# quokka-astro/quokka

Measured on AMD Instinct MI355X. Metric: Mcell-updates/s on 3D Sedov unigrid, higher is better.
Workload: dtype f64; 1 GPU; 3D Sedov blast 256x256x256 unigrid (tests/blast_unigrid_256.in scaled to 256^3 cells per GPU), 128^3 boxes, PPM+HLLC RK2, gamma=1.4, CFL 0.3, reflecting octant; cells_per_gpu=16777216, boxes_per_gpu=8, parallelism=box-decomposition x1, rk2_mode=carry, fofc_stages=0, retries=0, x_sweep_in_y_march=True

## Files before the change

include/quokka_amd.h:

```cpp
#ifndef QUOKKA_AMD_H_
#define QUOKKA_AMD_H_

#include <stdint.h>

#ifdef __cplusplus
extern "C" {
#endif

typedef struct qk_ctx qk_ctx;
typedef struct qk_level qk_level;
typedef void *qk_stream;

typedef enum qk_status {
	QK_OK = 0,
	QK_ERR_INVALID = -1,
	QK_ERR_HIP = -2,
	QK_ERR_UNSUPPORTED = -3,
	QK_ERR_STATE = -4
} qk_status;

typedef struct qk_array4 {
	double *p;
	int64_t jstride, kstride, nstride;
	int begin[3];
// ... 202 lines not shown
int qk_ghost_plan_destroy(qk_ghost_plan *plan);
int qk_ghost_plan_num_peers(qk_ghost_plan *plan);
int qk_ghost_plan_peer(qk_ghost_plan *plan, int k, int *rank, int64_t *send_count, int64_t *recv_count);
int qk_ghost_plan_num_items(qk_ghost_plan *plan, int kind, int k);
int qk_ghost_plan_item(qk_ghost_plan *plan, int kind, int k, int idx, int *dst_box, int *src_box, int lo[3], int hi[3], int shift[3], int64_t *offset);
int qk_FillBoundary_local(qk_ghost_plan *plan, qk_stream s, qk_array4 *state);
int qk_FillBoundary_local_int(qk_ghost_plan *plan, qk_stream s, qk_iarray4 *state);
int qk_FillBoundary_pack(qk_ghost_plan *plan, qk_stream s, int k, const qk_array4 *state, double *sendbuf);
int qk_FillBoundary_unpack(qk_ghost_plan *plan, qk_stream s, int k, qk_array4 *state, const double *recvbuf);
int qk_FillBoundary_pack_int(qk_ghost_plan *plan, qk_stream s, int k, const qk_iarray4 *state, int *sendbuf);
int qk_FillBoundary_unpack_int(qk_ghost_plan *plan, qk_stream s, int k, qk_iarray4 *state, const int *recvbuf);
int qk_SumBoundary_local(qk_ghost_plan *plan, qk_stream s, qk_array4 *state);
int qk_SumBoundary_pack(qk_ghost_plan *plan, qk_stream s, int k, const qk_array4 *state, double *buf);
int qk_SumBoundary_unpack(qk_ghost_plan *plan, qk_stream s, int k, qk_array4 *state, const double *buf);
int qk_FillPhysicalBoundary(qk_ghost_plan *plan, qk_stream s, qk_array4 *state, const qk_bcrec *bcs, const qk_dirichlet_face *dirichlet);
int qk_ghost_plan_set_components(qk_ghost_plan *plan, int scomp, int ncomp);
#define QK_BOXES_ALL 0
#define QK_BOXES_LOCAL_ONLY 1
#define QK_BOXES_REMOTE_DEPENDENT 2
int qk_ghost_plan_box_is_remote(qk_ghost_plan *plan, int local_box);
int qk_ghost_plan_set_box_remote(qk_ghost_plan *plan, int local_box, int flag);
int qk_FillPhysicalBoundary_subset(qk_ghost_plan *plan, qk_stream s, qk_array4 *state, const qk_bcrec *bcs, const qk_dirichlet_face *dirichlet,
				   int which);

typedef struct qk_carray4 {
	char *p;
	int64_t jstride, kstride, nstride;
	int begin[3];
	int end[3];
	int ncomp;
} qk_carray4;
enum { QK_TAG_CLEAR = 0, QK_TAG_BUF = 1, QK_TAG_SET = 2 };
#define QK_TAGFIELD_PRESSURE (-1)
int qk_tag_relative_gradient(qk_level *lev, qk_stream s, const qk_hydro_traits *t, const qk_array4 *state, qk_carray4 *tags, int field,
			     double eta_threshold, double q_min, int min_inclusive);
int qk_tag_centered_gradient(qk_level *lev, qk_stream s, const qk_array4 *state, qk_carray4 *tags, int comp, int dir, double dx, double eta_threshold,
			     double q_min, int min_inclusive);
int qk_PreInterpState(qk_level *lev, qk_stream s, qk_array4 *mf);
int qk_PostInterpState(qk_level *lev, qk_stream s, qk_array4 *mf);
typedef struct qk_avgdown_plan qk_avgdown_plan;
int qk_avgdown_plan_create(qk_level *crse, qk_level *fine, const int ratio[3], qk_avgdown_plan **plan);
int qk_avgdown_plan_destroy(qk_avgdown_plan *plan);
int qk_avgdown_plan_num_items(qk_avgdown_plan *plan);
int qk_average_down(qk_avgdown_plan *plan, qk_stream s, const qk_array4 *fine, qk_array4 *crse, int scomp, int ncomp);

typedef struct qk_interp_plan qk_interp_plan;
// ... 82 lines not shown
```

quokka_amd/capi.py:

```python
from __future__ import annotations

import ctypes as C
import os

_HERE = os.path.dirname(os.path.abspath(__file__))
LIB_PATH = os.environ.get("QK_LIB_PATH", os.path.join(_HERE, "lib", "libquokka_amd.so"))

QK_OK, QK_ERR_INVALID, QK_ERR_HIP, QK_ERR_UNSUPPORTED, QK_ERR_STATE = 0, -1, -2, -3, -4
ERR_UNSUPPORTED = QK_ERR_UNSUPPORTED
HOOK_COMPILED = 100
DIR_X1, DIR_X2, DIR_X3 = 0, 1, 2
ARITH_DIVBY_RECIPOF, ARITH_DIVN, ARITH_RECIPEXACT, ARITH_SQRTN = 0, 1, 2, 3
RIEMANN_HLLC, RIEMANN_LLF, RIEMANN_HLLD = 0, 1, 2
LIMITER_MINMOD, LIMITER_MC = 0, 1
BC_REFLECT_ODD, BC_INT_DIR, BC_REFLECT_EVEN, BC_FOEXTRAP, BC_EXT_DIR = -1, 0, 1, 2, 3

K_B = 1.380649e-16
M_U = 1.6605390666e-24


class Array4(C.Structure):
    _fields_ = [("p", C.c_void_p), ("jstride", C.c_int64), ("kstride", C.c_int64), ("nstride", C.c_int64),
                ("begin", C.c_int * 3), ("end", C.c_int * 3), ("ncomp", C.c_int)]

# ... 46 lines not shown
        for g in range(ng + 1):
            self.rad_boundaries[g] = float(boundaries[g])
            self.mg_kappa_exponent[g] = float(kappa_exponent[g])
            self.mg_kappa_lower[g] = float(kappa_lower[g])
        self.mg_kappa_rho_exponent, self.mg_kappa_T_ref, self.mg_kappa_T_exponent = float(rho_exponent), float(T_ref), float(T_exponent)
        return self


class CloudyTables(C.Structure):
    _fields_ = [("log_nH", C.c_void_p), ("log_Tgas", C.c_void_p), ("cooling", C.c_void_p), ("heating", C.c_void_p), ("mean_mol_weight", C.c_void_p),
                ("n_nH", C.c_int), ("n_Tgas", C.c_int), ("T_min", C.c_double), ("T_max", C.c_double), ("mmw_min", C.c_double), ("mmw_max", C.c_double)]


class StageArgs(C.Structure):
    _fields_ = [("U_in", C.c_void_p), ("U_old", C.c_void_p), ("U_out", C.c_void_p),
                ("halfFlux", C.c_void_p * 3), ("halfVel", C.c_void_p * 3),
                ("redoFlag", C.c_void_p), ("d_redo_count", C.c_void_p), ("d_error_flag", C.c_void_p), ("d_max_signal", C.c_void_p),
                ("scratch", C.c_void_p), ("scratch_bytes", C.c_int64),
                ("dx", C.c_double * 3), ("dt", C.c_double), ("stage", C.c_int), ("reconstruction_order", C.c_int),
                ("densityFloor", C.c_double), ("tempFloor", C.c_double), ("use_dual_energy", C.c_int), ("K_visc", C.c_double),
                ("store_flux_rk2", C.c_int), ("fluxRk2", C.c_void_p * 3), ("rk2_carry_rhs", C.c_int), ("rhs1", C.c_void_p), ("flux_mask", C.c_void_p), ("fofc_pass", C.c_int),
                ("prim_out", C.c_int), ("prim_in", C.c_int),
                ("store_vel_rk2", C.c_int), ("velRk2", C.c_void_p * 3)]


def traits(gamma=1.4, reconstruct_eint=True, ndim=3, mean_molecular_weight=M_U, boltzmann_constant=K_B,
           cs_isothermal=float("nan"), nscalars=0, nmscalars=0, eos_temperature_model=0, eos_alpha=0.0) -> HydroTraits:
    return HydroTraits(gamma, cs_isothermal, mean_molecular_weight, boltzmann_constant, int(reconstruct_eint), nscalars, nmscalars, ndim,
                       int(eos_temperature_model), float(eos_alpha))


class QkError(RuntimeError):
    pass


_lib = None


def lib() -> C.CDLL:
    global _lib
    if _lib is not None:
        return _lib
    if not os.path.exists(LIB_PATH):
        raise QkError(f"{LIB_PATH} is missing: run `python -c 'import __graft_entry__ as g; g.build()'` "
                      "(hipcc --offload-arch=gfx950). The hot path has no CPU fallback.")
    L = C.CDLL(LIB_PATH)
# ... 33 lines not shown
    L.qk_hydro_EnforceLimits.argtypes = [vp, vp, T, cd, cd, vp]
    L.qk_hydro_SyncDualEnergy.argtypes = [vp, vp, T, vp, vp]
    L.qk_hydro_ComputeMaxSignalSpeed.argtypes = [vp, vp, T, vp, vp]
    L.qk_hydro_maxSignalSpeedLocal.argtypes = [vp, vp, T, ci, vp, vp]
    L.qk_replaceFluxes.argtypes = [vp, vp, ci, vp, vp, vp, ci]
    L.qk_Saxpy.argtypes = [vp, vp, ci, vp, cd, vp, ci]
    R = P(RadTraits)
    L.qk_rad_ConservedToPrimitive.argtypes = [vp, vp, R, vp, vp, ci]
    L.qk_rad_ComputeFluxes.argtypes = [vp, vp, R, ci, vp, vp, vp, vp, vp]
    L.qk_rad_computeRadiationFluxes.argtypes = [vp, vp, R, ci, ci, vp, P(vp), P(vp)]
    L.qk_rad_ComputeWavespeedCorrection.argtypes = [vp, vp, R, T, ci, vp, P(cd), P(vp)]
    L.qk_rad_PredictStep.argtypes = [vp, vp, R, ci, vp, vp, P(vp), cd, P(cd)]
    L.qk_rad_AddFluxesRK2.argtypes = [vp, vp, R, ci, vp, vp, vp, P(vp), P(vp), cd, P(cd)]
    L.qk_hydro_FixupState.argtypes = [vp, vp, T, cd, cd, ci, vp, vp, vp]
    L.qk_rad_stage_fused.argtypes = [vp, vp, R, ci, ci, vp, vp, vp, vp, P(vp), cd, P(cd), P(vp)]
    L.qk_rad_AddSourceTermsSingleGroup.argtypes = [vp, vp, R, T, vp, vp, cd, ci, vp, vp]
    L.qk_rad_AddSourceTermsSingleGroupMirror.argtypes = [vp, vp, R, T, vp, vp, cd, ci, vp, vp, vp]
    L.qk_rad_AddSourceTermsMultiGroup.argtypes = [vp, vp, R, T, vp, vp, cd, ci, vp, vp]
    L.qk_rad_mg_planck_fractions.argtypes = [vp, R, cd, ci, P(cd), P(cd), P(cd)]
    if hasattr(L, "qk_hydro_stage_fused"):
        L.qk_hydro_stage_scratch_bytes.argtypes = [vp, T]
        L.qk_hydro_stage_scratch_bytes.restype = C.c_int64
        L.qk_hydro_stage_fused.argtypes = [vp, vp, T, P(StageArgs)]
    if hasattr(L, "qk_ghost_plan_create"):
        L.qk_ghost_plan_create.argtypes = [vp, P(vp), P(Geometry), ci, ci, ci, P(Box), P(ci), ci]
        L.qk_ghost_plan_destroy.argtypes = [vp]
        L.qk_ghost_plan_num_peers.argtypes = [vp]
        L.qk_ghost_plan_peer.argtypes = [vp, ci, P(ci), P(C.c_int64), P(C.c_int64)]
        L.qk_ghost_plan_num_items.argtypes = [vp, ci, ci]
        L.qk_ghost_plan_item.argtypes = [vp, ci, ci, ci, P(ci), P(ci), ci * 3, ci * 3, ci * 3, P(C.c_int64)]
        L.qk_FillBoundary_local.argtypes = [vp, vp, vp]
        L.qk_FillBoundary_local_int.argtypes = [vp, vp, vp]
        L.qk_FillBoundary_pack.argtypes = [vp, vp, ci, vp, vp]
        L.qk_FillBoundary_unpack.argtypes = [vp, vp, ci, vp, vp]
        L.qk_SumBoundary_local.argtypes = [vp, vp, vp]
        L.qk_SumBoundary_pack.argtypes = [vp, vp, ci, vp, vp]
        L.qk_SumBoundary_unpack.argtypes = [vp, vp, ci, vp, vp]
        L.qk_FillBoundary_pack_int.argtypes = [vp, vp, ci, vp, vp]
        L.qk_FillBoundary_unpack_int.argtypes = [vp, vp, ci, vp, vp]
        L.qk_FillPhysicalBoundary.argtypes = [vp, vp, vp, P(BCRec), P(DirichletFace)]
        L.qk_FillPhysicalBoundary_subset.argtypes = [vp, vp, vp, P(BCRec), P(DirichletFace), C.c_int]
        L.qk_ghost_plan_set_components.argtypes = [vp, C.c_int, C.c_int]
        L.qk_ghost_plan_box_is_remote.argtypes = [vp, C.c_int]
        L.qk_ghost_plan_set_box_remote.argtypes = [vp, C.c_int, C.c_int]
    if hasattr(L, "qk_tag_relative_gradient"):
        L.qk_tag_relative_gradient.argtypes = [vp, vp, T, vp, vp, ci, C.c_double, C.c_double, ci]
# ... 26 lines not shown
        L.qk_PreInterpState.argtypes = [vp, vp, vp]
        L.qk_PostInterpState.argtypes = [vp, vp, vp]
        L.qk_fluxreg_create_crse_part.argtypes = [vp, vp, P(Geometry), ci * 3, ci, P(vp)]
        L.qk_pcopy_plan_create.argtypes = [vp, P(Geometry), ci, P(Box), P(ci), ci, ci, ci, P(Box), P(ci), ci, vp, ci, ci, P(vp)]
        L.qk_pcopy_plan_destroy.argtypes = [vp]
        L.qk_pcopy_plan_num_peers.argtypes = [vp]
        L.qk_pcopy_plan_peer.argtypes = [vp, ci, P(ci), P(C.c_int64), P(C.c_int64)]
        L.qk_pcopy_plan_num_items.argtypes = [vp, ci, ci]
        L.qk_pcopy_plan_item.argtypes = [vp, ci, ci, ci, P(ci), P(ci), ci * 3, ci * 3, ci * 3, P(C.c_int64)]
        L.qk_ParallelCopy_local.argtypes = [vp, vp, vp, vp, ci, ci, ci]
        L.qk_ParallelCopy_pack.argtypes = [vp, vp, ci, vp, ci, vp]
        L.qk_ParallelCopy_unpack.argtypes = [vp, vp, ci, vp, ci, vp, ci]
    L.qk_tracer_plan_create.argtypes = [vp, P(vp), P(Geometry), cd * 3, cd * 3, cd * 3]
    L.qk_tracer_plan_destroy.argtypes = [vp]
    L.qk_tracer_plan_lattice.argtypes = [vp, ci * 3, P(C.c_int64)]
    L.qk_tracer_InitOnePerCell.argtypes = [vp, vp, cd * 3, vp * 3, vp * 3, vp, vp, C.c_int64, ci]
    L.qk_tracer_AdvectWithUmac.argtypes = [vp, vp, vp * 3, cd, C.c_int64, vp * 3, vp * 3]
    L.qk_tracer_Redistribute.argtypes = [vp, vp, C.c_int64, vp * 3, vp]
    _lib = L
    return L


BOXES_ALL, BOXES_LOCAL_ONLY, BOXES_REMOTE_DEPENDENT = 0, 1, 2
TAG_CLEAR, TAG_BUF, TAG_SET = 0, 1, 2
TAGFIELD_PRESSURE = -1

DECLARED_SYMBOLS = [
    "qk_ctx_create", "qk_ctx_destroy", "qk_last_error", "qk_version", "qk_level_create", "qk_level_destroy",
    "qk_upload_array4_table", "qk_upload_iarray4_table", "qk_clear_bytes", "qk_profile_enable", "qk_profile_only", "qk_profile_reset", "qk_profile_num_kernels", "qk_profile_get",
    "qk_ReconstructStatesConstant", "qk_ReconstructStatesPLM", "qk_ReconstructStatesPPM",
    "qk_hydro_ConservedToPrimitive", "qk_hydro_ComputeFlatteningCoefficients", "qk_hydro_FlattenShocks",
    "qk_hydro_ComputeFluxes", "qk_hydro_ComputeRhsFromFluxes", "qk_hydro_AddInternalEnergyPdV", "qk_hydro_PredictStep",
    "qk_hydro_EnforceLimits", "qk_hydro_SyncDualEnergy", "qk_hydro_ComputeMaxSignalSpeed", "qk_hydro_maxSignalSpeedLocal",
    "qk_replaceFluxes", "qk_Saxpy", "qk_hydro_FixupState", "qk_hydro_stage_scratch_bytes", "qk_hydro_stage_fused",
    "qk_rad_ConservedToPrimitive", "qk_rad_ComputeWavespeedCorrection", "qk_rad_ComputeFluxes", "qk_rad_computeRadiationFluxes", "qk_rad_PredictStep", "qk_rad_AddFluxesRK2", "qk_rad_stage_fused",
    "qk_rad_AddSourceTermsSingleGroup", "qk_rad_AddSourceTermsSingleGroupMirror", "qk_rad_AddSourceTermsMultiGroup", "qk_rad_mg_planck_fractions",
    "qk_ghost_plan_create", "qk_ghost_plan_destroy", "qk_ghost_plan_num_peers", "qk_ghost_plan_peer", "qk_ghost_plan_num_items", "qk_ghost_plan_item",
    "qk_FillBoundary_local", "qk_FillBoundary_local_int", "qk_FillBoundary_pack", "qk_FillBoundary_unpack", "qk_FillBoundary_pack_int", "qk_FillBoundary_unpack_int", "qk_SumBoundary_local", "qk_SumBoundary_pack", "qk_SumBoundary_unpack", "qk_FillPhysicalBoundary",
    "qk_FillPhysicalBoundary_subset", "qk_ghost_plan_set_components", "qk_ghost_plan_box_is_remote", "qk_ghost_plan_set_box_remote",
    "qk_tag_relative_gradient", "qk_tag_centered_gradient", "qk_avgdown_plan_create", "qk_avgdown_plan_destroy", "qk_avgdown_plan_num_items", "qk_average_down", "qk_PreInterpState", "qk_PostInterpState",
    "qk_interp_plan_create", "qk_interp_plan_destroy", "qk_interp_plan_num_items", "qk_interp_plan_item", "qk_InterpFromCoarse",
    "qk_fluxreg_create", "qk_fluxreg_destroy", "qk_fluxreg_num_items", "qk_fluxreg_item", "qk_fluxreg_reset", "qk_fluxreg_save", "qk_fluxreg_restore", "qk_fluxreg_CrseAdd", "qk_fluxreg_FineAdd",
    "qk_fluxreg_Reflux", "qk_fluxreg_set_state_component", "qk_amr_tile_flags", "qk_amr_tile_flags_periodic", "qk_amr_cluster_tiles", "qk_amr_cluster_berger_rigoutsos", "qk_copy_box",
    "qk_cloudy_tables_read", "qk_cloudy_tables_free", "qk_cooling_tabulated", "qk_cooling_evaluate", "qk_arith_evaluate",
    "qk_fluxreg_create_crse_part", "qk_pcopy_plan_create", "qk_pcopy_plan_destroy", "qk_pcopy_plan_num_peers", "qk_pcopy_plan_peer", "qk_pcopy_plan_num_items",
    "qk_pcopy_plan_item", "qk_ParallelCopy_local", "qk_ParallelCopy_pack", "qk_ParallelCopy_unpack",
    "qk_tracer_plan_create", "qk_tracer_plan_destroy", "qk_tracer_plan_lattice", "qk_tracer_InitOnePerCell", "qk_tracer_AdvectWithUmac", "qk_tracer_Redistribute",
]


def check(ctx, rc: int, what: str = "") -> None:
    if rc != QK_OK:
        msg = lib().qk_last_error(ctx).decode() if ctx else ""
        raise QkError(f"{what} failed with status {rc}: {msg}")
```

quokka_amd/csrc/qk_boundary.hip:

```cpp
#include <algorithm>
#include <cstdlib>
#include <array>
#include <map>
#include <cstring>
#include <vector>

#include "qk_device.hpp"
#include "qk_internal.hpp"

using namespace qk;

namespace
{

struct CopyItem {
	int dst_box;
	int src_box;
	int lo[3], hi[3];
	int shift[3];
	int64_t offset;
};

struct PeerPlan {
	int rank = -1;
// ... 9 lines not shown
}

}

struct qk_ghost_plan {
	qk_level *lev = nullptr;
	qk_geometry geom{};
	int nghost = 0, ncomp = 0;
	std::vector<CopyItem> local;
	CopyItem *d_local = nullptr;
	int max_local_cells = 0;
	std::vector<PeerPlan> peers;
	std::vector<CopyItem> shells;
	CopyItem *d_shells = nullptr;
	int max_shell_cells = 0;
	int n_shells_indep = 0;
	std::vector<char> box_remote;
	int active_scomp = 0, active_ncomp = -1;
	void *d_physbc = nullptr;
	std::vector<unsigned char> h_physbc;
	qk_bcrec *d_bcs = nullptr;
	int d_bcs_n = 0;
	qk_dirichlet_face *d_dir = nullptr;
};

namespace
{

void partitionShells(qk_ghost_plan *P)
{
	auto indep = [&](CopyItem const &it) { return P->box_remote[it.dst_box] == 0; };
	std::stable_partition(P->shells.begin(), P->shells.end(), indep);
	P->n_shells_indep = static_cast<int>(std::count_if(P->shells.begin(), P->shells.end(), indep));
}

enum CopyMode { MODE_LOCAL = 0, MODE_PACK = 1, MODE_UNPACK = 2, MODE_SUM_LOCAL = 3, MODE_SUM_PACK = 4, MODE_SUM_UNPACK = 5 };

template <int MODE, typename T = double, typename D = qk_array4>
__global__ void __launch_bounds__(256) k_copy(const CopyItem *items, const D *state_t, T *buf, int ncomp, int scomp = 0)
{
	const CopyItem it = items[blockIdx.y];
	const unsigned n0 = static_cast<unsigned>(it.hi[0] - it.lo[0] + 1), n1 = static_cast<unsigned>(it.hi[1] - it.lo[1] + 1),
		       n2 = static_cast<unsigned>(it.hi[2] - it.lo[2] + 1);
	const unsigned n01 = n0 * n1;
	const unsigned ncell = n01 * n2;
	const unsigned total = ncell * static_cast<unsigned>(ncomp);
// ... 129 lines not shown
			for (int d = 0; d < 3; ++d) {
				if (side[d] == 0) {
					continue;
				}
				const int type = (side[d] < 0) ? bc.lo[d] : bc.hi[d];
				const int edge = (side[d] < 0) ? geom.domain.lo[d] : geom.domain.hi[d];
				if (type == QK_BC_FOEXTRAP) {
					src[d] = edge;
					any = true;
				} else if (type == QK_BC_REFLECT_EVEN || type == QK_BC_REFLECT_ODD) {
					src[d] = (side[d] < 0) ? (2 * edge - idx[d] - 1) : (2 * edge - idx[d] + 1);
					neg = neg != (type == QK_BC_REFLECT_ODD);
					any = true;
				}
			}
			if (any) {
				const double v = A(src[0], src[1], src[2], n);
				A(idx[0], idx[1], idx[2], n) = neg ? -v : v;
			}
		}
	}
}

auto uploadItems(qk_ctx *ctx, std::vector<CopyItem> const &v, CopyItem **d) -> int
{
	*d = nullptr;
	if (v.empty() || ctx->device < 0) {
		return QK_OK;
	}
	QK_HIP_CHECK(ctx, hipMalloc(reinterpret_cast<void **>(d), sizeof(CopyItem) * v.size()));
	QK_HIP_CHECK(ctx, hipMemcpy(*d, v.data(), sizeof(CopyItem) * v.size(), hipMemcpyHostToDevice));
	return QK_OK;
}

inline auto gridFor(int64_t cells, int nitems) -> dim3
{
	const int64_t gx = std::max<int64_t>(1, std::min<int64_t>((cells + 255) / 256, 256));
	return dim3(static_cast<unsigned>(gx), static_cast<unsigned>(nitems), 1);
}
constexpr int MAX_ITEMS_PER_LAUNCH = 65535;

template <class Launch> void forItemChunks(int count, Launch &&launch)
{
	for (int a = 0; a < count; a += MAX_ITEMS_PER_LAUNCH) {
		launch(a, std::min(count - a, MAX_ITEMS_PER_LAUNCH));
	}
// ... 177 lines not shown
	}
	if (rc != QK_OK) {
		qk_ghost_plan_destroy(P);
		return rc;
	}
	*plan_out = P;
	return QK_OK;
}

int qk_ghost_plan_destroy(qk_ghost_plan *plan)
{
	if (plan == nullptr) {
		return QK_ERR_INVALID;
	}
	(void)hipFree(plan->d_local);
	(void)hipFree(plan->d_shells);
	for (auto &p : plan->peers) {
		(void)hipFree(p.d_send);
		(void)hipFree(p.d_recv);
	}
	(void)hipFree(plan->d_bcs);
	(void)hipFree(plan->d_dir);
	(void)hipFree(plan->d_physbc);
	delete plan;
	return QK_OK;
}

int qk_ghost_plan_num_peers(qk_ghost_plan *plan) { return plan == nullptr ? QK_ERR_INVALID : static_cast<int>(plan->peers.size()); }

int qk_ghost_plan_peer(qk_ghost_plan *plan, int k, int *rank, int64_t *send_count, int64_t *recv_count)
{
	if (plan == nullptr) {
		return QK_ERR_INVALID;
	}
	QK_REQUIRE(plan->lev->ctx, k >= 0 && k < static_cast<int>(plan->peers.size()) && rank && send_count && recv_count, "qk_ghost_plan_peer: bad index");
	*rank = plan->peers[k].rank;
	*send_count = plan->peers[k].send_count;
	*recv_count = plan->peers[k].recv_count;
	return QK_OK;
}

static auto planItems(qk_ghost_plan *plan, int kind, int k) -> std::vector<CopyItem> const *
{
	if (kind == 0) {
		return &plan->local;
	}
// ... 204 lines not shown
	QK_HIP_CHECK(ctx, hipGetLastError());
	return QK_OK;
}

int qk_ghost_plan_box_is_remote(qk_ghost_plan *plan, int local_box)
{
	if (plan == nullptr || local_box < 0 || local_box >= plan->lev->nboxes) {
		return QK_ERR_INVALID;
	}
	return plan->box_remote[local_box];
}

int qk_ghost_plan_set_box_remote(qk_ghost_plan *plan, int local_box, int flag)
{
	if (plan == nullptr || local_box < 0 || local_box >= plan->lev->nboxes) {
		return QK_ERR_INVALID;
	}
	qk_ctx *ctx = plan->lev->ctx;
	plan->box_remote[local_box] = (flag != 0) ? 1 : 0;
	partitionShells(plan);
	if (plan->d_shells != nullptr && !plan->shells.empty()) {
		QK_HIP_CHECK(ctx, hipMemcpy(plan->d_shells, plan->shells.data(), sizeof(CopyItem) * plan->shells.size(), hipMemcpyHostToDevice));
	}
	return QK_OK;
}

int qk_FillPhysicalBoundary(qk_ghost_plan *plan, qk_stream s, qk_array4 *state_t, const qk_bcrec *bcs, const qk_dirichlet_face *dirichlet)
{
	return qk_FillPhysicalBoundary_subset(plan, s, state_t, bcs, dirichlet, QK_BOXES_ALL);
}

int qk_ghost_plan_set_components(qk_ghost_plan *plan, int scomp, int ncomp)
{
	if (plan == nullptr) {
		return QK_ERR_INVALID;
	}
	QK_REQUIRE(plan->lev->ctx, ncomp < 0 || (scomp >= 0 && ncomp >= 1 && scomp + ncomp <= plan->ncomp), "ghost_plan_set_components: bad range");
	plan->active_scomp = (ncomp < 0) ? 0 : scomp;
	plan->active_ncomp = ncomp;
	return QK_OK;
}

int qk_FillPhysicalBoundary_subset(qk_ghost_plan *plan, qk_stream s, qk_array4 *state_t, const qk_bcrec *bcs, const qk_dirichlet_face *dirichlet,
				   int which)
{
	if (plan == nullptr) {
// ... 64 lines not shown
```

quokka_amd/simulation.py:

```python
from __future__ import annotations

import ctypes as C
import math
import os
from dataclasses import dataclass
from typing import Callable, List, Optional, Sequence, Tuple

import numpy as np
import torch

from . import capi
from .hydro_system import HydroSystem, HyperbolicSystem, Saxpy, replaceFluxes
from .multifab import Context, Level, MultiFab

NGHOST_CC = 4


def chop_domain(n_cell: Sequence[int], max_grid_size: Sequence[int]) -> List[Tuple[List[int], List[int]]]:
    nb = [(n_cell[d] + max_grid_size[d] - 1) // max_grid_size[d] for d in range(3)]
    boxes = []
    for kb in range(nb[2]):
        for jb in range(nb[1]):
            for ib in range(nb[0]):
                lo, hi = [], []
# ... 98 lines not shown
        self.peers = []
        for k in range(L.qk_ghost_plan_num_peers(h)):
            r, ns, nr = C.c_int(), C.c_int64(), C.c_int64()
            ctx.check(L.qk_ghost_plan_peer(h, k, C.byref(r), C.byref(ns), C.byref(nr)), "qk_ghost_plan_peer")
            self.peers.append((k, r.value, torch.empty(ns.value, dtype=dtype, device=ctx.device), torch.empty(nr.value, dtype=dtype, device=ctx.device)))

    def fill(self, state: MultiFab, between=None, before_physbc=None):
        ctx = self.lev.ctx
        L = ctx.L
        s = ctx.stream()
        def pack(k, sbuf):
            ctx.check(L.qk_FillBoundary_pack(self.h, s, k, state.ptr, C.c_void_p(sbuf.data_ptr())), "FillBoundary_pack")

        def local():
            ctx.check(L.qk_FillBoundary_local(self.h, s, state.ptr), "FillBoundary_local")

        def unpack(k, rbuf):
            ctx.check(L.qk_FillBoundary_unpack(self.h, s, k, state.ptr, C.c_void_p(rbuf.data_ptr())), "FillBoundary_unpack")

        def physbc(which):
            ctx.check(L.qk_FillPhysicalBoundary_subset(self.h, s, state.ptr, self.bcs, self.dirichlet, which), "FillPhysicalBoundary")

        self.fill_with(pack, local, unpack, physbc, between, before_physbc)

    def fill_with(self, pack, local, unpack, physbc, between=None, before_physbc=None):
        pending = None
        if self.peers:
            from . import comm
            for k, r, sbuf, rbuf in self.peers:
                pack(k, sbuf)
            pending = comm.exchange([(r, sbuf, rbuf) for k, r, sbuf, rbuf in self.peers])
        local()
        bc = not self.geom.is_all_periodic()
        if between is not None:
            if bc:
                physbc(capi.BOXES_LOCAL_ONLY)
            between()
        if pending is not None:
            if self.exposed_events is not None:
                e0, e1 = torch.cuda.Event(enable_timing=True), torch.cuda.Event(enable_timing=True)
                e0.record()
                pending.wait()
                e1.record()
                self.exposed_events.append((e0, e1))
            else:
                pending.wait()
# ... 84 lines not shown
        self.min_overlap_cells = 8 * 128 ** 3
        self.use_fused = use_fused and traits.nscalars <= 3 and traits.nmscalars == 0
        lev = self.lev
        self.state_old_cc_ = MultiFab(lev, self.ncomp_cc, NGHOST_CC, fill=0.0)
        self.state_new_cc_ = MultiFab(lev, self.ncomp_cc, NGHOST_CC, fill=0.0)
        self.state_old_tmp = MultiFab(lev, self.ncomp_cc, NGHOST_CC, fill=0.0)
        self.state_inter_cc_ = MultiFab(lev, self.ncomp_cc, NGHOST_CC, fill=0.0)
        self.tNew_ = 0.0
        self.dt_ = 1.0e100
        self.istep = 0
        self.cellUpdates_ = 0
        self.counters = {"fofc1_stages": 0, "fofc2_stages": 0, "retries": 0}
        self.strang_sources = []
        self.ghost = GhostExchange(lev, geom, self.ncomp_cc, NGHOST_CC, self.all_boxes, self.owner, rank, bcs, dirichlet)
        self.flag_ghost = None
        nd = geom.ndim
        self.halfFlux = [MultiFab(lev, self.hydro.nvar_, 0, facedir=d) for d in range(nd)]
        self.halfVel = [MultiFab(lev, 1, 0, facedir=d) for d in range(nd)]
        self.redoFlag = MultiFab(lev, 1, 1, dtype=torch.int32, fill=0)
        self._dev_words = torch.zeros(8, dtype=torch.int64, device=ctx.device)
        self.speculate_stage2 = True
        self.prim_handoff = os.environ.get("QK_PRIM_HANDOFF", "1") == "1"
        self._prim_now = False
        self._has_dirichlet = dirichlet is not None
        self.dev_counters = self._dev_words[2:3]
        self.dev_error = self._dev_words[3:4].view(torch.int32)[0:1]
        self._err_latched = False
        self._unfused_ran = False
        self.dev_max = torch.zeros(1, dtype=torch.float64, device=ctx.device)
        self.dev_signal = self._dev_words[0:2].view(torch.float64)
        self._dev_fix = torch.zeros(8, dtype=torch.int64, device=ctx.device)
        self._fix_far_words = False
        self._fix_words_pending = False
        self._signal_of_state_new = None
        self.scratch = None
        if self.use_fused:
            nbytes = ctx.L.qk_hydro_stage_scratch_bytes(lev.h, C.byref(traits))
            assert nbytes > 0 or not self.my_boxes
            self.scratch = torch.empty(max(nbytes // 8, 1), dtype=torch.float64, device=ctx.device)
        self._unfused_tmp = None

    def CountCells(self) -> int:
        return sum(int(np.prod([hi[d] - lo[d] + 1 for d in range(3)])) for lo, hi in self.all_boxes)

    def fillBoundaryConditions(self, state: MultiFab):
        self.ghost.fill(state)
# ... 243 lines not shown
    def rhs1(self):
        if getattr(self, "_rhs1", None) is None:
            self._rhs1 = MultiFab(self.lev, self.hydro.nvar_ + 1, 0, fill=0.0)
        return self._rhs1

    def _prim_handoff_applies(self) -> bool:
        return type(self) is HydroSimulation and self._prim_handoff_state_ok()

    def _prim_handoff_state_ok(self) -> bool:
        t = self.traits
        return (self.prim_handoff and not self._has_dirichlet and self.ncomp_cc == self.hydro.nvar_
                and t.reconstruct_eint == 0 and t.cs_isothermal != t.cs_isothermal and t.eos_temperature_model == 0 and t.gamma != 1.0)

    def _is_final(self, stage: int) -> bool:
        return (stage == 2) or (self.integratorOrder_ == 1)

    def _fused_begin(self, stage: int, slot: int = 0, both: bool = False):
        if self._unfused_ran and not self._err_latched:
            self._err_latched = int(self.dev_error.item()) != 0
        c = self.ctx
        c.check(c.L.qk_clear_bytes(c.h, c.stream(), C.c_void_p(self._dev_words.data_ptr() + (0 if both else 32 * slot)), 64 if both else 32), "qk_clear_bytes")

    def _fused_launch(self, stage: int, U_in, U_old, U_out, dt, group=None, fofc: bool = False, slot: int = 0, scratch=None):
        lev, idx = (self.lev, None) if group is None else group
        tab = (lambda mf: mf.ptr) if idx is None else (lambda mf: mf.subset_ptr(idx))
        a = capi.StageArgs()
        a.U_in, a.U_old, a.U_out = tab(U_in), tab(U_old), tab(U_out)
        nd = self.geom.ndim
        for d in range(3):
            a.halfFlux[d] = tab(self.halfFlux[d]) if d < nd else None
            a.halfVel[d] = tab(self.halfVel[d]) if d < nd else None
            a.dx[d] = self.geom.dx[d] if d < nd else 1.0
        a.redoFlag = tab(self.redoFlag)
        w = self._dev_words.data_ptr() + 32 * slot
        a.d_redo_count = C.c_void_p(w + 16)
        a.d_error_flag = C.c_void_p(w + 24)
        if self._is_final(stage):
            a.d_max_signal = C.c_void_p(w)
        sc = self.scratch if scratch is None else scratch
        a.scratch = C.c_void_p(sc.data_ptr())
        a.scratch_bytes = sc.numel() * 8
        a.dt, a.stage, a.reconstruction_order = dt, stage, self.reconstructionOrder_
        a.densityFloor, a.tempFloor, a.use_dual_energy, a.K_visc = self.densityFloor_, self.tempFloor_, self.useDualEnergy_, float(self.artificialViscosityK_)
        mask = getattr(self, "flux_mask", None)
        if self._carry_active():
            a.rk2_carry_rhs = 1
            a.rhs1 = tab(self.rhs1())
            if mask is not None:
                a.flux_mask = tab(mask)
        else:
            a.store_flux_rk2 = int(self._needs_flux_rk2())
        if a.store_flux_rk2 or a.flux_mask:
            for d in range(nd):
                a.fluxRk2[d] = tab(self.fluxRk2()[d])
        if stage == 2 and self._tracers_on_fused():
            a.store_vel_rk2 = 1
            for d in range(nd):
                a.velRk2[d] = tab(self.velRk2()[d])
        a.fofc_pass = int(fofc)
        if self._prim_now and not fofc:
            a.prim_out, a.prim_in = int(stage == 1), int(stage == 2)
        c = self.ctx
        c.check(c.L.qk_hydro_stage_fused(lev.h, c.stream(), C.byref(self.traits), C.byref(a)), "qk_hydro_stage_fused")

    def _read_words(self):
        if self.nranks > 1:
            import torch.distributed as dist
            from . import comm
            w = self._dev_words.view(2, 4)
            v = torch.cat([w[:, 0:2].reshape(-1).view(torch.float64).view(2, 2), w[:, 2:3].to(torch.float64),
                           (w[:, 3:4] & 0xFFFFFFFF).to(torch.float64)], dim=1).reshape(-1)
            comm.all_reduce(v, dist.ReduceOp.MAX)
            vals = v.tolist()
            return [vals[0:4], vals[4:8]]
        hw = self.__dict__.get("_host_words")
        if hw is None:
            hw = self.__dict__["_host_words"] = torch.zeros(8, dtype=torch.int64).pin_memory()
            self.__dict__["_host_words_np"] = hw.numpy()
        hw.copy_(self._dev_words, non_blocking=True)
        torch.cuda.current_stream(self.ctx.device).synchronize()
        a = self.__dict__["_host_words_np"]
        f = a.view(np.float64)
        return [[float(f[4 * s]), float(f[4 * s + 1]), float(a[4 * s + 2]), float(int(a[4 * s + 3]) & 0xFFFFFFFF)] for s in (0, 1)]

    def _fused_end(self, stage: int, slot: int = 0, vals=None) -> int:
        final = self._is_final(stage)
        vals = (self._read_words() if vals is None else vals)[slot]
        self._err_latched = self._err_latched or vals[3] != 0.0
        nbad = int(vals[2])
        if final and nbad == 0:
            self._signal_of_state_new = (vals[0], vals[1])
        return nbad

    def overlap_groups(self):
        late = self.ghost.remote_boxes()
        key = tuple(late)
        if getattr(self, "_groups_key", None) != key:
            early = [b for b in range(self.lev.nboxes) if b not in set(late)]
            self._groups = None
            cells = lambda idx: sum(int(np.prod([self.my_boxes[b][1][d] - self.my_boxes[b][0][d] + 1 for d in range(3)])) for b in idx)
            if early and late and min(cells(early), cells(late)) >= self.min_overlap_cells:
                mk = lambda idx: (Level(self.ctx, self.geom.ndim, [self.my_boxes[b] for b in idx]), idx)
                self._groups = (mk(early), mk(late))
            self._groups_key = key
# ... 96 lines not shown
        for src in self.strang_sources:
            ok = src(state, time, dt) and ok
        return ok

    def advanceHydroAtLevel(self, state_old_tmp: MultiFab, dt_lev: float, time: Optional[float] = None) -> bool:
        time = (self.tNew_ - self.dt_) if time is None else time
        if self.strang_sources and not self._strang_sources(state_old_tmp, time, 0.5 * dt_lev):
            return False
        self._signal_of_state_new = None
        self._err_latched, self._unfused_ran = False, False
        with_tracers = bool(self.do_tracers) and self.tracers is not None
        if with_tracers:
            self._check_tracers()
        fused = self.use_fused and (not with_tracers or self._tracers_on_fused())
        self._avg_face_vel = None
        pair_done = False
        self._prim_now = False
        if getattr(self, "_prim_backoff", 0) > 0:
            self._prim_backoff -= 1
        elif fused and self.integratorOrder_ == 2 and self.speculate_stage2 and self._prim_handoff_applies():
            inter, new = self.state_inter_cc_, self.state_new_cc_
            self._prim_now = True
            try:
                self._fused_begin(1, both=True)
                self._launch_stage(1, state_old_tmp, state_old_tmp, inter, dt_lev, slot=0)
                self._launch_stage(2, inter, state_old_tmp, new, dt_lev, slot=1)
            finally:
                self._prim_now = False
            vals = self._read_words()
            latched = self._err_latched
            if self._fused_end(1, 0, vals) == 0 and self._fused_end(2, 1, vals) == 0:
                self._stage1_left_F1 = not self._carry_active()
                self._fused_stage_stood(2)
                pair_done = True
                self._prim_backoff_len = 0
            else:
                self._prim_backoff_len = min(64, max(4, 2 * getattr(self, "_prim_backoff_len", 0)))
                self._prim_backoff = self._prim_backoff_len
                self._err_latched = latched
                self._signal_of_state_new = None
                self.counters["prim_handoff_dropped"] = self.counters.get("prim_handoff_dropped", 0) + 1
        if pair_done:
            pass
        elif fused and self.integratorOrder_ == 2 and self.speculate_stage2:
            inter, new = self.state_inter_cc_, self.state_new_cc_
            self._fused_begin(1, both=True)
            self._launch_stage(1, state_old_tmp, state_old_tmp, inter, dt_lev, slot=0)
            self._launch_stage(2, inter, state_old_tmp, new, dt_lev, slot=1)
            vals = self._read_words()
            if self._fused_end(1, 0, vals) == 0:
                self._stage1_left_F1 = not self._carry_active()
                if not self._finish_stage(2, inter, state_old_tmp, new, dt_lev, self._fused_end(2, 1, vals)):
                    return False
                pair_done = True
            else:
                self._err_latched = False
        if pair_done:
            pass
        elif not self._fill_and_stage(1, state_old_tmp, state_old_tmp, self.state_inter_cc_, dt_lev, fused):
            return False
        elif self.integratorOrder_ == 2:
            if not self._fill_and_stage(2, self.state_inter_cc_, state_old_tmp, self.state_new_cc_, dt_lev, fused):
                return False
        else:
            for b in range(self.lev.nboxes):
                self.state_new_cc_.valid(b)[0:6].copy_(self.state_inter_cc_.valid(b)[0:6])
        if self._err_latched or (self._unfused_ran and int(self.dev_error.item()) != 0):
            raise capi.QkError("density is negative in SyncDualEnergy! abort!! (reference src/hydro/hydro_system.hpp:834-836)")
        if with_tracers:
            if self._avg_face_vel is None:
                raise capi.QkError("do_tracers: no stage 2 of this advance left avgFaceVel behind")
            self.tracers.advect(self._avg_face_vel, dt_lev)
        if self.strang_sources:
            ok = self._strang_sources(self.state_new_cc_, time + dt_lev, 0.5 * dt_lev)
# ... 297 lines not shown
```

Measured before the change: 3203 Mcell-updates/s.

## Add native RK2 step entry point with single-launch ghost gather fill

Adds a C entry point that runs ghost fill, stage 1, ghost fill, and stage 2 of the RK2 step in one host call. It also adds a precomputed gather plan that fills interior copies and physical (reflect/extrapolate) boundaries in a single kernel launch instead of separate local-copy and physical-boundary passes. The goal is to cut Python/ctypes dispatch and kernel-launch overhead per step and drop a boundary pass. It adds plan-building complexity, and it falls back to the old path when the boundaries mix modes, when Dirichlet faces are present, or when there are remote peers.

```diff
diff --git a/include/quokka_amd.h b/include/quokka_amd.h
--- a/include/quokka_amd.h
+++ b/include/quokka_amd.h
@@ -248,6 +248,19 @@
 int qk_ghost_plan_set_box_remote(qk_ghost_plan *plan, int local_box, int flag);
 int qk_FillPhysicalBoundary_subset(qk_ghost_plan *plan, qk_stream s, qk_array4 *state, const qk_bcrec *bcs, const qk_dirichlet_face *dirichlet,
 				   int which);
+#define QK_GATHER_NOT_APPLICABLE 1
+int qk_FillBoundary_gather(qk_ghost_plan *plan, qk_stream s, qk_array4 *state, const qk_bcrec *bcs);
+
+typedef struct qk_hydro_step_args {
+	const qk_hydro_stage_args *stage1, *stage2;
+	qk_ghost_plan *ghost;
+	const qk_bcrec *bcs;
+	void *d_verdict;
+	void *h_verdict;
+	int64_t verdict_bytes;
+	int one_launch_fill;
+} qk_hydro_step_args;
+int qk_hydro_step_rk2(qk_level *lev, qk_stream s, const qk_hydro_traits *t, const qk_hydro_step_args *a);
 
 typedef struct qk_carray4 {
 	char *p;
diff --git a/quokka_amd/capi.py b/quokka_amd/capi.py
--- a/quokka_amd/capi.py
+++ b/quokka_amd/capi.py
@@ -92,6 +92,11 @@
                 ("store_flux_rk2", C.c_int), ("fluxRk2", C.c_void_p * 3), ("rk2_carry_rhs", C.c_int), ("rhs1", C.c_void_p), ("flux_mask", C.c_void_p), ("fofc_pass", C.c_int),
                 ("prim_out", C.c_int), ("prim_in", C.c_int),
                 ("store_vel_rk2", C.c_int), ("velRk2", C.c_void_p * 3)]
+
+
+class StepArgs(C.Structure):
+    _fields_ = [("stage1", C.POINTER(StageArgs)), ("stage2", C.POINTER(StageArgs)), ("ghost", C.c_void_p), ("bcs", C.POINTER(BCRec)),
+                ("d_verdict", C.c_void_p), ("h_verdict", C.c_void_p), ("verdict_bytes", C.c_int64), ("one_launch_fill", C.c_int)]
 
 
 def traits(gamma=1.4, reconstruct_eint=True, ndim=3, mean_molecular_weight=M_U, boltzmann_constant=K_B,
@@ -171,6 +176,8 @@
         L.qk_hydro_stage_scratch_bytes.argtypes = [vp, T]
         L.qk_hydro_stage_scratch_bytes.restype = C.c_int64
         L.qk_hydro_stage_fused.argtypes = [vp, vp, T, P(StageArgs)]
+    L.qk_hydro_step_rk2.argtypes = [vp, vp, T, P(StepArgs)]
+    L.qk_FillBoundary_gather.argtypes = [vp, vp, vp, P(BCRec)]
     if hasattr(L, "qk_ghost_plan_create"):
         L.qk_ghost_plan_create.argtypes = [vp, P(vp), P(Geometry), ci, ci, ci, P(Box), P(ci), ci]
         L.qk_ghost_plan_destroy.argtypes = [vp]
@@ -243,6 +250,7 @@
 
 
 BOXES_ALL, BOXES_LOCAL_ONLY, BOXES_REMOTE_DEPENDENT = 0, 1, 2
+GATHER_NOT_APPLICABLE = 1
 TAG_CLEAR, TAG_BUF, TAG_SET = 0, 1, 2
 TAGFIELD_PRESSURE = -1
 
@@ -259,6 +267,7 @@
     "qk_ghost_plan_create", "qk_ghost_plan_destroy", "qk_ghost_plan_num_peers", "qk_ghost_plan_peer", "qk_ghost_plan_num_items", "qk_ghost_plan_item",
     "qk_FillBoundary_local", "qk_FillBoundary_local_int", "qk_FillBoundary_pack", "qk_FillBoundary_unpack", "qk_FillBoundary_pack_int", "qk_FillBoundary_unpack_int", "qk_SumBoundary_local", "qk_SumBoundary_pack", "qk_SumBoundary_unpack", "qk_FillPhysicalBoundary",
     "qk_FillPhysicalBoundary_subset", "qk_ghost_plan_set_components", "qk_ghost_plan_box_is_remote", "qk_ghost_plan_set_box_remote",
+    "qk_FillBoundary_gather", "qk_hydro_step_rk2",
     "qk_tag_relative_gradient", "qk_tag_centered_gradient", "qk_avgdown_plan_create", "qk_avgdown_plan_destroy", "qk_avgdown_plan_num_items", "qk_average_down", "qk_PreInterpState", "qk_PostInterpState",
     "qk_interp_plan_create", "qk_interp_plan_destroy", "qk_interp_plan_num_items", "qk_interp_plan_item", "qk_InterpFromCoarse",
     "qk_fluxreg_create", "qk_fluxreg_destroy", "qk_fluxreg_num_items", "qk_fluxreg_item", "qk_fluxreg_reset", "qk_fluxreg_save", "qk_fluxreg_restore", "qk_fluxreg_CrseAdd", "qk_fluxreg_FineAdd",
diff --git a/quokka_amd/csrc/qk_boundary.hip b/quokka_amd/csrc/qk_boundary.hip
--- a/quokka_amd/csrc/qk_boundary.hip
+++ b/quokka_amd/csrc/qk_boundary.hip
@@ -55,6 +55,11 @@
 	qk_bcrec *d_bcs = nullptr;
 	int d_bcs_n = 0;
 	qk_dirichlet_face *d_dir = nullptr;
+	void *d_gather = nullptr, *d_gather_blocks = nullptr;
+	int n_gather = 0, n_gather_blocks = 0;
+	int64_t max_gather_cells = 0;
+	int gather_state = 0;
+	std::vector<qk_bcrec> gather_bcs;
 };
 
 namespace
@@ -230,6 +235,243 @@
 	}
 }
 
+struct GatherItem {
+	int dst_box, src_box;
+	int lo[3], hi[3];
+	int a[3], b[3];
+	unsigned long long neg;
+};
+
+struct GatherBlock {
+	int item, chunk, nchunks;
+};
+
+__global__ void __launch_bounds__(256) k_gather(const GatherItem *items, const GatherBlock *blocks, qk_array4 *state_t, int ncomp, int scomp)
+{
+	const GatherBlock gb = blocks[blockIdx.x];
+	const GatherItem it = items[gb.item];
+	const unsigned n0 = static_cast<unsigned>(it.hi[0] - it.lo[0] + 1), n1 = static_cast<unsigned>(it.hi[1] - it.lo[1] + 1),
+		       n2 = static_cast<unsigned>(it.hi[2] - it.lo[2] + 1);
+	const unsigned n01 = n0 * n1;
+	const unsigned ncell = n01 * n2;
+	const unsigned total = ncell * static_cast<unsigned>(ncomp);
+	A4<double, qk_array4> Dst(state_t[it.dst_box]);
+	A4<double, qk_array4> Src(state_t[it.src_box]);
+	const unsigned stride = static_cast<unsigned>(gb.nchunks) * 256u;
+	for (unsigned t = static_cast<unsigned>(gb.chunk) * 256u + threadIdx.x; t < total; t += stride) {
+		const unsigned un = t / ncell;
+		const unsigned c = t - un * ncell;
+		const unsigned uk = c / n01;
+		const unsigned r = c - uk * n01;
+		const unsigned uj = r / n0;
+		const int n = scomp + static_cast<int>(un);
+		const int di = it.lo[0] + static_cast<int>(r - uj * n0), dj = it.lo[1] + static_cast<int>(uj), dk = it.lo[2] + static_cast<int>(uk);
+		const double v = Src(it.a[0] * di + it.b[0], it.a[1] * dj + it.b[1], it.a[2] * dk + it.b[2], n);
+		Dst(di, dj, dk, n) = (((it.neg >> n) & 1ull) != 0) ? -v : v;
+	}
+}
+
+auto buildGather(qk_ghost_plan *P, const qk_bcrec *bcs) -> int
+{
+	qk_ctx *ctx = P->lev->ctx;
+	qk_level *lev = P->lev;
+	const qk_geometry &geom = P->geom;
+	P->gather_bcs.assign(bcs, bcs + P->ncomp);
+	P->gather_state = 2;
+	if (P->d_gather != nullptr) {
+		QK_HIP_CHECK(ctx, hipFree(P->d_gather));
+		QK_HIP_CHECK(ctx, hipFree(P->d_gather_blocks));
+		P->d_gather = nullptr;
+		P->d_gather_blocks = nullptr;
+	}
+	if (!P->peers.empty() || P->ncomp > 64) {
+		return QK_OK;
+	}
+	int mode[3][2];
+	unsigned long long odd[3][2];
+	for (int d = 0; d < 3; ++d) {
+		for (int sd = 0; sd < 2; ++sd) {
+			mode[d][sd] = -1;
+			odd[d][sd] = 0;
+			if (d >= geom.ndim || geom.periodic[d] != 0) {
+				continue;
+			}
+			for (int n = 0; n < P->ncomp; ++n) {
+				const int type = (sd == 0) ? bcs[n].lo[d] : bcs[n].hi[d];
+				const int m = (type == QK_BC_REFLECT_EVEN || type == QK_BC_REFLECT_ODD) ? 1 : (type == QK_BC_FOEXTRAP ? 2 : 0);
+				if (mode[d][sd] == -1) {
+					mode[d][sd] = m;
+				} else if (mode[d][sd] != m) {
+					mode[d][sd] = 0;
+				}
+				if (type == QK_BC_REFLECT_ODD) {
+					odd[d][sd] |= 1ull << n;
+				}
+			}
+		}
+	}
+	std::vector<GatherItem> items;
+	for (auto const &c : P->local) {
+		GatherItem g{};
+		g.dst_box = c.dst_box;
+		g.src_box = c.src_box;
+		for (int d = 0; d < 3; ++d) {
+			g.lo[d] = c.lo[d];
+			g.hi[d] = c.hi[d];
+			g.a[d] = 1;
+			g.b[d] = -c.shift[d];
+		}
+		items.push_back(g);
+	}
+	for (int b = 0; b < lev->nboxes; ++b) {
+		qk_box grown = lev->boxes[b];
+		for (int d = 0; d < geom.ndim; ++d) {
+			grown.lo[d] -= P->nghost;
+			grown.hi[d] += P->nghost;
+		}
+		struct Piece {
+			int src_box, lo[3], hi[3], shift[3];
+		};
+		std::vector<Piece> pieces;
+		{
+			Piece own{};
+			own.src_box = b;
+			for (int d = 0; d < 3; ++d) {
+				own.lo[d] = lev->boxes[b].lo[d];
+				own.hi[d] = lev->boxes[b].hi[d];
+			}
+			pieces.push_back(own);
+			for (auto const &c : P->local) {
+				if (c.dst_box == b) {
+					Piece q{};
+					q.src_box = c.src_box;
+					for (int d = 0; d < 3; ++d) {
+						q.lo[d] = c.lo[d];
+						q.hi[d] = c.hi[d];
+						q.shift[d] = c.shift[d];
+					}
+					pieces.push_back(q);
+				}
+			}
+		}
+		for (int oz = -1; oz <= 1; ++oz) {
+			for (int oy = -1; oy <= 1; ++oy) {
+				for (int ox = -1; ox <= 1; ++ox) {
+					const int o[3] = {ox, oy, oz};
+					if (ox == 0 && oy == 0 && oz == 0) {
+						continue;
+					}
+					int slo[3], shi[3], a[3], bb[3];
+					unsigned long long neg = 0;
+					bool ok = true, applies = true;
+					for (int d = 0; d < 3 && ok; ++d) {
+						const bool wall = d < geom.ndim && geom.periodic[d] == 0;
+						if (o[d] != 0 && !wall) {
+							ok = false;
+						} else if (o[d] < 0) {
+							slo[d] = grown.lo[d];
+							shi[d] = std::min(grown.hi[d], geom.domain.lo[d] - 1);
+						} else if (o[d] > 0) {
+							slo[d] = std::max(grown.lo[d], geom.domain.hi[d] + 1);
+							shi[d] = grown.hi[d];
+						} else {
+							slo[d] = wall ? std::max(grown.lo[d], geom.domain.lo[d]) : grown.lo[d];
+							shi[d] = wall ? std::min(grown.hi[d], geom.domain.hi[d]) : grown.hi[d];
+						}
+						ok = ok && shi[d] >= slo[d];
+						if (ok && o[d] != 0) {
+							const int sd = (o[d] > 0) ? 1 : 0;
+							const int edge = (sd == 0) ? geom.domain.lo[d] : geom.domain.hi[d];
+							if (mode[d][sd] == 1) {
+								a[d] = -1;
+								bb[d] = (sd == 0) ? (2 * edge - 1) : (2 * edge + 1);
+								neg ^= odd[d][sd];
+							} else if (mode[d][sd] == 2) {
+								a[d] = 0;
+								bb[d] = edge;
+							} else {
+								applies = false;
+							}
+						} else if (ok) {
+							a[d] = 1;
+							bb[d] = 0;
+						}
+					}
+					if (!ok) {
+						continue;
+					}
+					if (!applies) {
+						return QK_OK;
+					}
+					int64_t want = 1, have = 0;
+					for (int d = 0; d < 3; ++d) {
+						want *= shi[d] - slo[d] + 1;
+					}
+					for (auto const &pc : pieces) {
+						GatherItem g{};
+						g.dst_box = b;
+						g.src_box = pc.src_box;
+						g.neg = neg;
+						bool hit = true;
+						for (int d = 0; d < 3 && hit; ++d) {
+							if (a[d] == 1) {
+								g.lo[d] = std::max(slo[d], pc.lo[d]);
+								g.hi[d] = std::min(shi[d], pc.hi[d]);
+							} else if (a[d] == -1) {
+								const int ilo = bb[d] - shi[d], ihi = bb[d] - slo[d];
+								const int jlo = std::max(ilo, pc.lo[d]), jhi = std::min(ihi, pc.hi[d]);
+								g.lo[d] = bb[d] - jhi;
+								g.hi[d] = bb[d] - jlo;
+							} else {
+								g.lo[d] = slo[d];
+								g.hi[d] = (bb[d] >= pc.lo[d] && bb[d] <= pc.hi[d]) ? shi[d] : slo[d] - 1;
+							}
+							hit = g.hi[d] >= g.lo[d];
+							g.a[d] = a[d];
+							g.b[d] = bb[d] - pc.shift[d];
+						}
+						if (hit) {
+							have += regionCells(CopyItem{0, 0, {g.lo[0], g.lo[1], g.lo[2]}, {g.hi[0], g.hi[1], g.hi[2]}, {0, 0, 0}, 0});
+							items.push_back(g);
+						}
+					}
+					if (have != want) {
+						return QK_OK;
+					}
+				}
+			}
+		}
+	}
+	if (items.empty()) {
+		return QK_OK;
+	}
+	int64_t biggest = 0;
+	for (auto const &g : items) {
+		biggest = std::max<int64_t>(biggest, static_cast<int64_t>(g.hi[0] - g.lo[0] + 1) * (g.hi[1] - g.lo[1] + 1) * (g.hi[2] - g.lo[2] + 1));
+	}
+	if (biggest * P->ncomp >= (int64_t{1} << 31)) {
+		return QK_OK;
+	}
+	std::vector<GatherBlock> blocks;
+	for (size_t k = 0; k < items.size(); ++k) {
+		auto const &g = items[k];
+		const int64_t values = static_cast<int64_t>(g.hi[0] - g.lo[0] + 1) * (g.hi[1] - g.lo[1] + 1) * (g.hi[2] - g.lo[2] + 1) * P->ncomp;
+		const int nchunks = static_cast<int>((values + 2047) / 2048);
+		for (int c = 0; c < nchunks; ++c) {
+			blocks.push_back({static_cast<int>(k), c, nchunks});
+		}
+	}
+	QK_HIP_CHECK(ctx, hipMalloc(&P->d_gather, sizeof(GatherItem) * items.size()));
+	QK_HIP_CHECK(ctx, hipMemcpy(P->d_gather, items.data(), sizeof(GatherItem) * items.size(), hipMemcpyHostToDevice));
+	QK_HIP_CHECK(ctx, hipMalloc(&P->d_gather_blocks, sizeof(GatherBlock) * blocks.size()));
+	QK_HIP_CHECK(ctx, hipMemcpy(P->d_gather_blocks, blocks.data(), sizeof(GatherBlock) * blocks.size(), hipMemcpyHostToDevice));
+	P->n_gather_blocks = static_cast<int>(blocks.size());
+	P->n_gather = static_cast<int>(items.size());
+	P->max_gather_cells = biggest;
+	P->gather_state = 1;
+	return QK_OK;
+}
+
 auto uploadItems(qk_ctx *ctx, std::vector<CopyItem> const &v, CopyItem **d) -> int
 {
 	*d = nullptr;
@@ -453,6 +695,8 @@
 	(void)hipFree(plan->d_bcs);
 	(void)hipFree(plan->d_dir);
 	(void)hipFree(plan->d_physbc);
+	(void)hipFree(plan->d_gather);
+	(void)hipFree(plan->d_gather_blocks);
 	delete plan;
 	return QK_OK;
 }
@@ -703,6 +947,35 @@
 	if (plan->d_shells != nullptr && !plan->shells.empty()) {
 		QK_HIP_CHECK(ctx, hipMemcpy(plan->d_shells, plan->shells.data(), sizeof(CopyItem) * plan->shells.size(), hipMemcpyHostToDevice));
 	}
+	return QK_OK;
+}
+
+int qk_FillBoundary_gather(qk_ghost_plan *plan, qk_stream s, qk_array4 *state_t, const qk_bcrec *bcs)
+{
+	if (plan == nullptr) {
+		return QK_ERR_INVALID;
+	}
+	qk_ctx *ctx = plan->lev->ctx;
+	QK_REQUIRE(ctx, state_t && bcs, "FillBoundary_gather: NULL argument");
+	if (ctx->device < 0) {
+		return QK_GATHER_NOT_APPLICABLE;
+	}
+	if (plan->gather_state == 0 || std::memcmp(plan->gather_bcs.data(), bcs, sizeof(qk_bcrec) * plan->ncomp) != 0) {
+		if (plan->gather_state == 1) {
+			QK_HIP_CHECK(ctx, hipStreamSynchronize(static_cast<hipStream_t>(s)));
+		}
+		if (int rc = buildGather(plan, bcs); rc != QK_OK) {
+			return rc;
+		}
+	}
+	if (plan->gather_state != 1) {
+		return QK_GATHER_NOT_APPLICABLE;
+	}
+	const int nc = (plan->active_ncomp < 0) ? plan->ncomp : plan->active_ncomp;
+	ProfScope ps(ctx, static_cast<hipStream_t>(s), "ghost_gather");
+	hipLaunchKernelGGL(k_gather, dim3(static_cast<unsigned>(plan->n_gather_blocks)), dim3(256), 0, static_cast<hipStream_t>(s),
+			   static_cast<const GatherItem *>(plan->d_gather), static_cast<const GatherBlock *>(plan->d_gather_blocks), state_t, nc, plan->active_scomp);
+	QK_HIP_CHECK(ctx, hipGetLastError());
 	return QK_OK;
 }
 
diff --git a/quokka_amd/csrc/qk_hydro_step.hip b/quokka_amd/csrc/qk_hydro_step.hip
--- /dev/null
+++ b/quokka_amd/csrc/qk_hydro_step.hip
@@ -0,0 +1,59 @@
+#include "qk_internal.hpp"
+
+using namespace qk;
+
+namespace
+{
+
+auto fillGhosts(const qk_hydro_step_args *a, qk_stream s, const qk_array4 *state) -> int
+{
+	auto *st = const_cast<qk_array4 *>(state);
+	if (a->one_launch_fill != 0) {
+		const int rc = qk_FillBoundary_gather(a->ghost, s, st, a->bcs);
+		if (rc != QK_GATHER_NOT_APPLICABLE) {
+			return rc;
+		}
+	}
+	if (int rc = qk_FillBoundary_local(a->ghost, s, st); rc != QK_OK) {
+		return rc;
+	}
+	return qk_FillPhysicalBoundary(a->ghost, s, st, a->bcs, nullptr);
+}
+
+}
+
+extern "C" {
+
+int qk_hydro_step_rk2(qk_level *lev, qk_stream stream, const qk_hydro_traits *t, const qk_hydro_step_args *a)
+{
+	if (lev == nullptr) {
+		return QK_ERR_INVALID;
+	}
+	qk_ctx *ctx = lev->ctx;
+	QK_REQUIRE(ctx, a != nullptr && a->stage1 != nullptr && a->stage2 != nullptr && a->ghost != nullptr && a->bcs != nullptr, "qk_hydro_step_rk2: NULL argument");
+	QK_REQUIRE(ctx, a->stage1->stage == 1 && a->stage2->stage == 2, "qk_hydro_step_rk2: stage1 / stage2 must be the argument blocks of stage 1 and stage 2");
+	QK_REQUIRE(ctx, a->stage1->fofc_pass == 0 && a->stage2->fofc_pass == 0, "qk_hydro_step_rk2: no correction pass (the host redoes a flagged step)");
+	QK_REQUIRE(ctx, a->stage1->U_in != nullptr && a->stage2->U_in != nullptr, "qk_hydro_step_rk2: NULL state");
+	QK_REQUIRE(ctx, a->d_verdict != nullptr && a->verdict_bytes > 0, "qk_hydro_step_rk2: NULL verdict words");
+	QK_REQUIRE(ctx, qk_ghost_plan_num_peers(a->ghost) == 0, "qk_hydro_step_rk2: boxes on other ranks (the host's early / late exchange handles them)");
+	auto s = static_cast<hipStream_t>(stream);
+	QK_HIP_CHECK(ctx, hipMemsetAsync(a->d_verdict, 0, static_cast<size_t>(a->verdict_bytes), s));
+	if (int rc = fillGhosts(a, stream, a->stage1->U_in); rc != QK_OK) {
+		return rc;
+	}
+	if (int rc = qk_hydro_stage_fused(lev, stream, t, a->stage1); rc != QK_OK) {
+		return rc;
+	}
+	if (int rc = fillGhosts(a, stream, a->stage2->U_in); rc != QK_OK) {
+		return rc;
+	}
+	if (int rc = qk_hydro_stage_fused(lev, stream, t, a->stage2); rc != QK_OK) {
+		return rc;
+	}
+	if (a->h_verdict != nullptr) {
+		QK_HIP_CHECK(ctx, hipMemcpyAsync(a->h_verdict, a->d_verdict, static_cast<size_t>(a->verdict_bytes), hipMemcpyDeviceToHost, s));
+	}
+	return QK_OK;
+}
+
+}
diff --git a/quokka_amd/simulation.py b/quokka_amd/simulation.py
--- a/quokka_amd/simulation.py
+++ b/quokka_amd/simulation.py
@@ -144,6 +144,16 @@
             ctx.check(L.qk_FillPhysicalBoundary_subset(self.h, s, state.ptr, self.bcs, self.dirichlet, which), "FillPhysicalBoundary")
 
         self.fill_with(pack, local, unpack, physbc, between, before_physbc)
+
+    def fill_gather(self, state: MultiFab) -> bool:
+        ctx = self.lev.ctx
+        if self.dirichlet is not None:
+            return False
+        rc = ctx.L.qk_FillBoundary_gather(self.h, ctx.stream(), state.ptr, self.bcs)
+        if rc == capi.GATHER_NOT_APPLICABLE:
+            return False
+        ctx.check(rc, "qk_FillBoundary_gather")
+        return True
 
     def fill_with(self, pack, local, unpack, physbc, between=None, before_physbc=None):
         pending = None
@@ -274,6 +284,9 @@
         self.speculate_stage2 = True
         self.prim_handoff = os.environ.get("QK_PRIM_HANDOFF", "1") == "1"
         self._prim_now = False
+        self.native_step = os.environ.get("QK_NATIVE_STEP", "1") == "1"
+        self.native_gather = os.environ.get("QK_NATIVE_GATHER", "1") == "1"
+        self.native_steps_taken = 0
         self._has_dirichlet = dirichlet is not None
         self.dev_counters = self._dev_words[2:3]
         self.dev_error = self._dev_words[3:4].view(torch.int32)[0:1]
@@ -563,7 +576,13 @@
         c.check(c.L.qk_clear_bytes(c.h, c.stream(), C.c_void_p(self._dev_words.data_ptr() + (0 if both else 32 * slot)), 64 if both else 32), "qk_clear_bytes")
 
     def _fused_launch(self, stage: int, U_in, U_old, U_out, dt, group=None, fofc: bool = False, slot: int = 0, scratch=None):
-        lev, idx = (self.lev, None) if group is None else group
+        lev = self.lev if group is None else group[0]
+        a = self._stage_args(stage, U_in, U_old, U_out, dt, group, fofc, slot, scratch)
+        c = self.ctx
+        c.check(c.L.qk_hydro_stage_fused(lev.h, c.stream(), C.byref(self.traits), C.byref(a)), "qk_hydro_stage_fused")
+
+    def _stage_args(self, stage: int, U_in, U_old, U_out, dt, group=None, fofc: bool = False, slot: int = 0, scratch=None) -> capi.StageArgs:
+        idx = None if group is None else group[1]
         tab = (lambda mf: mf.ptr) if idx is None else (lambda mf: mf.subset_ptr(idx))
         a = capi.StageArgs()
         a.U_in, a.U_old, a.U_out = tab(U_in), tab(U_old), tab(U_out)
@@ -601,10 +620,37 @@
         a.fofc_pass = int(fofc)
         if self._prim_now and not fofc:
             a.prim_out, a.prim_in = int(stage == 1), int(stage == 2)
+        return a
+
+    def _native_step_applies(self) -> bool:
+        return (self.native_step and type(self) is HydroSimulation and self.nranks == 1 and not self._has_dirichlet and not self.ghost.peers
+                and getattr(self, "flux_mask", None) is None and self.overlap_groups() is None)
+
+    def _host_words(self):
+        hw = self.__dict__.get("_host_words_t")
+        if hw is None:
+            hw = self.__dict__["_host_words_t"] = torch.zeros(8, dtype=torch.int64).pin_memory()
+            self.__dict__["_host_words_np"] = hw.numpy()
+        return hw, self.__dict__["_host_words_np"]
+
+    def _launch_pair(self, U_old, inter, new, dt) -> bool:
+        if not self._native_step_applies():
+            self._fused_begin(1, both=True)
+            self._launch_stage(1, U_old, U_old, inter, dt, slot=0)
+            self._launch_stage(2, inter, U_old, new, dt, slot=1)
+            return False
+        a1 = self._stage_args(1, U_old, U_old, inter, dt, slot=0)
+        a2 = self._stage_args(2, inter, U_old, new, dt, slot=1)
+        sa = capi.StepArgs()
+        sa.stage1, sa.stage2 = C.pointer(a1), C.pointer(a2)
+        sa.ghost, sa.bcs = self.ghost.h, C.cast(self.ghost.bcs, C.POINTER(capi.BCRec))
+        sa.d_verdict, sa.h_verdict, sa.verdict_bytes = self._dev_words.data_ptr(), self._host_words()[0].data_ptr(), 64
+        sa.one_launch_fill = int(self.native_gather)
         c = self.ctx
-        c.check(c.L.qk_hydro_stage_fused(lev.h, c.stream(), C.byref(self.traits), C.byref(a)), "qk_hydro_stage_fused")
-
-    def _read_words(self):
+        c.check(c.L.qk_hydro_step_rk2(self.lev.h, c.stream(), C.byref(self.traits), C.byref(sa)), "qk_hydro_step_rk2")
+        return True
+
+    def _read_words(self, copied: bool = False):
         if self.nranks > 1:
             import torch.distributed as dist
             from . import comm
@@ -614,13 +660,10 @@
             comm.all_reduce(v, dist.ReduceOp.MAX)
             vals = v.tolist()
             return [vals[0:4], vals[4:8]]
-        hw = self.__dict__.get("_host_words")
-        if hw is None:
-            hw = self.__dict__["_host_words"] = torch.zeros(8, dtype=torch.int64).pin_memory()
-            self.__dict__["_host_words_np"] = hw.numpy()
-        hw.copy_(self._dev_words, non_blocking=True)
+        hw, a = self._host_words()
+        if not copied:
+            hw.copy_(self._dev_words, non_blocking=True)
         torch.cuda.current_stream(self.ctx.device).synchronize()
-        a = self.__dict__["_host_words_np"]
         f = a.view(np.float64)
         return [[float(f[4 * s]), float(f[4 * s + 1]), float(a[4 * s + 2]), float(int(a[4 * s + 3]) & 0xFFFFFFFF)] for s in (0, 1)]
 
@@ -763,14 +806,13 @@
             inter, new = self.state_inter_cc_, self.state_new_cc_
             self._prim_now = True
             try:
-                self._fused_begin(1, both=True)
-                self._launch_stage(1, state_old_tmp, state_old_tmp, inter, dt_lev, slot=0)
-                self._launch_stage(2, inter, state_old_tmp, new, dt_lev, slot=1)
+                native = self._launch_pair(state_old_tmp, inter, new, dt_lev)
             finally:
                 self._prim_now = False
-            vals = self._read_words()
+            vals = self._read_words(copied=native)
             latched = self._err_latched
             if self._fused_end(1, 0, vals) == 0 and self._fused_end(2, 1, vals) == 0:
+                self.native_steps_taken += int(native)
                 self._stage1_left_F1 = not self._carry_active()
                 self._fused_stage_stood(2)
                 pair_done = True
@@ -785,12 +827,11 @@
             pass
         elif fused and self.integratorOrder_ == 2 and self.speculate_stage2:
             inter, new = self.state_inter_cc_, self.state_new_cc_
-            self._fused_begin(1, both=True)
-            self._launch_stage(1, state_old_tmp, state_old_tmp, inter, dt_lev, slot=0)
-            self._launch_stage(2, inter, state_old_tmp, new, dt_lev, slot=1)
-            vals = self._read_words()
+            native = self._launch_pair(state_old_tmp, inter, new, dt_lev)
+            vals = self._read_words(copied=native)
             if self._fused_end(1, 0, vals) == 0:
                 self._stage1_left_F1 = not self._carry_active()
+                self.native_steps_taken += int(native and int(vals[1][2]) == 0)
                 if not self._finish_stage(2, inter, state_old_tmp, new, dt_lev, self._fused_end(2, 1, vals)):
                     return False
                 pair_done = True
```

Measured after the change: 3213 Mcell-updates/s (median of 6 runs). Within noise of the previous version (+0.3%).
